# jcatalang/LUDVM

Measured on AMD Instinct MI355X. Metric: biot_savart_pair_interactions_per_s, higher is better.
Workload: dtype f32

## Files before the change

include/ludvm_hip.h:

```cpp
#ifndef LUDVM_HIP_H
#define LUDVM_HIP_H

#include <stddef.h>

#ifdef __cplusplus
extern "C" {
#endif

#define LUDVM_ABI_VERSION 7

enum {
  LUDVM_OK = 0,
  LUDVM_E_ARG = 1,
  LUDVM_E_HIP = 2,
  LUDVM_E_NOMEM = 3,
  LUDVM_E_NODEVICE = 4,
  LUDVM_E_STATE = 5,
  LUDVM_E_COMM = 6
};

enum {
  LUDVM_PREC_F32 = 0,
  LUDVM_PREC_F32X2 = 1,
  LUDVM_PREC_F64 = 2
// ... 1 lines not shown

typedef struct ludvm_ctx ludvm_ctx;


int ludvm_abi_version(void);
int ludvm_create(int device_ordinal, ludvm_ctx** out);
int ludvm_destroy(ludvm_ctx* ctx);
const char* ludvm_last_error(const ludvm_ctx* ctx);
int ludvm_device_info(ludvm_ctx* ctx, int* cu_count, int* clock_khz, long long* hbm_bytes, char* name,
                      int name_len);
int ludvm_set_stream(ludvm_ctx* ctx, void* hip_stream, int external);
int ludvm_synchronize(ludvm_ctx* ctx);
int ludvm_set_tuning(ludvm_ctx* ctx, int targets_per_lane, int source_splits);

int ludvm_set_symmetric(ludvm_ctx* ctx, int mode);
int ludvm_set_sym_tuning(ludvm_ctx* ctx, int vortices_per_lane, int rotation_split);

typedef int (*ludvm_allreduce_fn)(void* user, void* d_buf, size_t count, void* hip_stream);
int ludvm_set_shard(ludvm_ctx* ctx, int rank, int world, size_t min_vortices, ludvm_allreduce_fn allreduce, void* user,
                    void* d_acc, size_t acc_bytes);

#define LUDVM_COMM_ID_BYTES 128
int ludvm_comm_unique_id(void* id_out, size_t id_bytes);
int ludvm_comm_init(ludvm_ctx* ctx, int rank, int world, const void* id, size_t id_bytes, size_t min_vortices);
int ludvm_comm_init_all(ludvm_ctx** ctxs, int n, size_t min_vortices);
int ludvm_comm_destroy(ludvm_ctx* ctx);
int ludvm_comm_info(ludvm_ctx* ctx, int* rank, int* world);
int ludvm_comm_allreduce_i64_dev(ludvm_ctx* ctx, long long* d_buf, size_t count);
int ludvm_comm_allgather_dev(ludvm_ctx* ctx, const void* d_send, void* d_recv, size_t bytes_per_rank);
int ludvm_comm_allgather_host(ludvm_ctx* ctx, const void* send, void* recv, size_t bytes_per_rank);
// ... 161 lines not shown
```

ludvm_amd/_ffi.py:

```python
import ctypes
import importlib.util
import os
import sys
from ctypes import POINTER, c_char_p, c_double, c_float, c_int, c_longlong, c_size_t, c_void_p

_HERE = os.path.dirname(os.path.abspath(__file__))
LIB_PATH = os.path.join(_HERE, "csrc", "libludvm_hip.so")
EXP_LIB_PATH = os.path.join(_HERE, "csrc", "libludvm_hip_exp.so")

OK, E_ARG, E_HIP, E_NOMEM, E_NODEVICE, E_STATE, E_COMM = range(7)
PREC_F32, PREC_F32X2, PREC_F64 = 0, 1, 2
SYM_TILE = 512
SYM_OWNER_ALIGN = 4
ABI_VERSION = 7
COMM_ID_BYTES = 128
ENSEMBLE_MAX_STEPS = 2048
ENSEMBLE_MAX_WAKE = 8192
ENSEMBLE_MAX_SNAPSHOTS = 1024
ENSEMBLE_INIT_HEAD = 8
ENSEMBLE_DESC = 6
ENSEMBLE_MAX_PROBES = 1024
ENSEMBLE_PROBE_BYTES = 1 << 30
ENSEMBLE_MAX_TRACERS = 4096
ENSEMBLE_TRACER_BYTES = 1 << 30
# ... 10 lines not shown
SURVEY_F32_PER_LANE = 4
SYM_SCALE_BYTES = 32

_pd, _pf = POINTER(c_double), POINTER(c_float)

SIGNATURES = {
    "ludvm_abi_version": [],
    "ludvm_create": [c_int, POINTER(c_void_p)],
    "ludvm_destroy": [c_void_p],
    "ludvm_last_error": [c_void_p],
    "ludvm_device_info": [c_void_p, POINTER(c_int), POINTER(c_int), POINTER(c_longlong), c_char_p, c_int],
    "ludvm_set_stream": [c_void_p, c_void_p, c_int],
    "ludvm_synchronize": [c_void_p],
    "ludvm_set_tuning": [c_void_p, c_int, c_int],
    "ludvm_set_symmetric": [c_void_p, c_int],
    "ludvm_set_shard": [c_void_p, c_int, c_int, c_size_t, c_void_p, c_void_p, c_void_p, c_size_t],
    "ludvm_set_sym_tuning": [c_void_p, c_int, c_int],
    "ludvm_comm_unique_id": [c_void_p, c_size_t],
    "ludvm_comm_init": [c_void_p, c_int, c_int, c_void_p, c_size_t, c_size_t],
    "ludvm_comm_init_all": [POINTER(c_void_p), c_int, c_size_t],
    "ludvm_comm_destroy": [c_void_p],
    "ludvm_comm_info": [c_void_p, POINTER(c_int), POINTER(c_int)],
    "ludvm_comm_allreduce_i64_dev": [c_void_p, c_void_p, c_size_t],
    "ludvm_comm_allgather_dev": [c_void_p, c_void_p, c_void_p, c_size_t],
    "ludvm_comm_allgather_host": [c_void_p, c_void_p, c_void_p, c_size_t],
    "ludvm_induce_f64": [c_void_p, _pd, _pd, _pd, c_size_t, _pd, _pd, c_size_t, c_double, c_int, _pd, _pd],
    "ludvm_spatial_order": [c_void_p, _pd, _pd, c_size_t, POINTER(ctypes.c_uint), POINTER(c_int), _pd],
    "ludvm_induce_f32": [c_void_p, _pf, _pf, _pf, c_size_t, _pf, _pf, c_size_t, c_float, _pf, _pf],
    "ludvm_induce_dev_f32": [c_void_p, c_void_p, c_void_p, c_void_p, c_size_t, c_void_p, c_void_p, c_size_t,
                             c_float, c_void_p, c_void_p],
# ... 142 lines not shown
```

ludvm_amd/csrc/context.hip:

```cpp
#include "ctx.hpp"

namespace ludvm_host {

int fail(ludvm_ctx* c, int code, const std::string& msg) {
  if (c) c->err = msg;
  return code;
}

int fail_hip(ludvm_ctx* c, const char* what, hipError_t e) {
  return fail(c, e == hipErrorOutOfMemory ? LUDVM_E_NOMEM : LUDVM_E_HIP,
              std::string(what) + ": " + hipGetErrorString(e));
}

int ensure(ludvm_ctx* c, Buf& b, size_t bytes) {
  if (bytes <= b.cap) return LUDVM_OK;
  HIPCHK(c, hipStreamSynchronize(c->stream));
  if (c->stream_b) HIPCHK(c, hipStreamSynchronize(c->stream_b));
  if (b.p) HIPCHK(c, hipFree(b.p));
  b.p = nullptr;
  b.cap = 0;
  size_t want = std::max(bytes, (size_t)1 << 20);
  HIPCHK(c, hipMalloc(&b.p, want));
  b.cap = want;
  return LUDVM_OK;
// ... 173 lines not shown
  c->shard_min_n = (long long)min_vortices;
  c->reduce_hook = world > 1 ? allreduce : nullptr;
  c->reduce_user = user;
  c->ext_acc = world > 1 ? d_acc : nullptr;
  c->ext_acc_bytes = world > 1 ? acc_bytes : 0;
  return LUDVM_OK;
}

int ludvm_set_symmetric(ludvm_ctx* c, int mode) {
  if (!c) return LUDVM_E_ARG;
  if (mode < 0) return fail(c, LUDVM_E_ARG, "symmetric mode must be >= 0");
  c->sym_mode = mode;
  return LUDVM_OK;
}

}
```

ludvm_amd/csrc/ctx.hpp:

```cpp
#pragma once
#pragma GCC visibility push(default)
#include "../../include/ludvm_hip.h"
#pragma GCC visibility pop
#include "pair_kernels.hpp"
#include "pair_sym_kernels.hpp"
#include "march_types.hpp"
#include "spatial_order.hpp"

#include <hip/hip_ext.h>
#include <rccl/rccl.h>
#include <dlfcn.h>

#include <algorithm>
#include <cmath>
#include <cstdio>
#include <cstdlib>
#include <cstring>
#include <string>
#include <utility>
#include <vector>

using namespace ludvm;

#ifdef LUDVM_EXPERIMENTS
// ... 9 lines not shown

struct TimedLaunch {
  hipEvent_t e0, e1;
};

struct ludvm_ctx {
  int device = 0;
  hipStream_t own_stream = nullptr;
  hipStream_t stream = nullptr;
  hipDeviceProp_t prop;
  std::string err;

  int tune_tpl = 0;
  int tune_split = 0;
  int sym_mode = 1;
  int tune_sym_t = 0, tune_sym_rsplit = 0;
  int xcd_run = 0;
  long long sym_tail_items = kSymTailItems;
  int grid_kernel = 2;
  long long small_tile_max = kSmallTileMaxDefault;
  bool sym_quad = true;
  long long sym_quad_min_tiles = kSymQuadMinTiles;
  bool few_packed = true;
  long long small_tile_max_f64 = kSmallTileMaxF64Default;

  Buf part;
  Buf acc;
  Buf symsc;
  Buf arena;
  Buf orderws;
// ... 106 lines not shown
  long long chunk;
  long long nt_pad;
  dim3 grid;
};

Plan make_plan(const ludvm_ctx* c, long long nt_launch, long long ns, int precision, bool small_ok = true, long long plan_nt = 0,
               bool grid_patch = false);
int timed_begin(ludvm_ctx* c, TimedLaunch& t, bool& active);
int timed_end(ludvm_ctx* c, TimedLaunch& t, bool active);
int drain_timing(ludvm_ctx* c);
int launch_pair(ludvm_ctx* c, PairArgs a, const Plan& p, int precision, void* u, void* w);
int induce_device(ludvm_ctx* c, const PairArgs& a, long long nt, long long ns, int precision, void* u, void* w,
                  long long plan_nt = 0);
long long sym_threshold(const ludvm_ctx* c, bool march = false);
bool use_symmetric(const ludvm_ctx* c, long long n, double vc4, bool march = false);
int sym_tile_t(const ludvm_ctx* c, long long n, bool hilo);

struct SymOperands {
  const float* x; const float* z; const float* g;
  const float* xl = nullptr; const float* zl = nullptr;
  const float* cx = nullptr; const float* cz = nullptr;
  long long* acc_u; long long* acc_w;
  const SymScale* scale; long long* bad;
};

int launch_sym_tiles(ludvm_ctx* c, int T, const SymOperands& o, long long n, long long i_first, long long i_count, double vc4,
                     const long long* n_dev = nullptr, long long n_lo = 0, bool sharded = false);
int acc_buffer(ludvm_ctx* c, long long nt_pad, long long** acc);
bool sharded_at(const ludvm_ctx* c, long long n);
void shard_tiles(const ludvm_ctx* c, long long ntiles, long long* first, long long* count);
// ... 13 lines not shown
  unsigned* order[2];
  double* ext;
  double* sum;
  void* tmp;
  size_t tmp_bytes;
};

int order_workspace(ludvm_ctx* c, size_t nmax, OrderWs* w);
int class_extent_sum(ludvm_ctx* c, const OrderWs& w, const double* dx, const double* dz, const unsigned* order, size_t n, double* out,
                     double* box = nullptr);
int spatial_order_if_needed(ludvm_ctx* c, const OrderWs& w, int slot, const double* dx, const double* dz, size_t n,
                            const unsigned** order_out, double* mean_extent);
int order_gather(ludvm_ctx* c, const double* s0, const double* s1, const double* s2, const unsigned* order, long long n, double* d0,
                 double* d1, double* d2);
int order_scatter(ludvm_ctx* c, const double* s0, const double* s1, const unsigned* order, long long n, double* d0, double* d1);
constexpr double kMaxExtentOverCore = 300.0;
constexpr double kMaxExtentOverCoreCloud = 150.0;
inline bool too_sparse(double mean_extent, bool reordered, double vcore) {
  return vcore > 0.0 && mean_extent > (reordered ? kMaxExtentOverCoreCloud : kMaxExtentOverCore) * vcore;
}

int wake_grow(ludvm_ctx* c, size_t capacity);
int wake_refresh(ludvm_ctx* c, size_t first, size_t count, bool staged = false);
inline unsigned fin_blocks(long long n) { return (unsigned)((n + kFinBlock - 1) / kFinBlock); }
struct MarchSym { const SymScale* scale = nullptr; long long* bad = nullptr; long long n_lo = 0; bool march = false; };
int advect_launch(ludvm_ctx* c, size_t n, const long long* n_dev, double dt, size_t nfoil, double vcore,
                  int precision, double* du, double* dw, TailDuty td = TailDuty{}, MarchSym ms = MarchSym{});

}

// ... 2 lines not shown
```

ludvm_amd/csrc/induce.hip:

```cpp
#include "ctx.hpp"
#include "induce_kernels.hpp"

extern "C" {


int ludvm_induce_f64(ludvm_ctx* c, const double* xs, const double* zs, const double* gs, size_t ns, const double* xt,
                     const double* zt, size_t nt, double vcore, int precision, double* u, double* w) {
  if (!c) return LUDVM_E_ARG;
  if (!valid_precision(precision)) return fail(c, LUDVM_E_ARG, "unknown precision");
  if ((ns && (!xs || !zs || !gs)) || (nt && (!xt || !zt || !u || !w))) return fail(c, LUDVM_E_ARG, "null array");
  if (nt == 0) return LUDVM_OK;
  HIPCHK(c, hipSetDevice(c->device));
  if (ns == 0) {
    std::memset(u, 0, nt * sizeof(double));
    std::memset(w, 0, nt * sizeof(double));
    return LUDVM_OK;
  }
  if (precision == LUDVM_PREC_F32 && std::min(ns, nt) < kOrderMin)
    precision = (double)ns * (double)nt <= kSmallSidePairsF64 ? LUDVM_PREC_F64 : LUDVM_PREC_F32X2;
  const bool f64 = precision == LUDVM_PREC_F64;
  bool hilo = precision == LUDVM_PREC_F32X2;
  const bool self = xt == xs && zt == zs && nt == ns;
  const size_t ntu = self ? 0 : nt;
  const size_t in_doubles = 3 * ns + 2 * ntu, out_doubles = 2 * nt;
// ... 77 lines not shown
    if (hilo)
      hipLaunchKernelGGL(cvt_packed_inputs, dim3(blocks_for((long long)in_doubles)), dim3(kBlock), 0, c->stream, din,
                         (long long)ns, (long long)ntu, fxs, fxsl, fzs, fzsl, fgs, fxt, fxtl, fzt, fztl);
    else
      hipLaunchKernelGGL(cvt_packed_inputs_local, dim3(blocks_for((long long)in_doubles)), dim3(kBlock), 0, c->stream, din,
                         (long long)ns, (long long)ntu, fxs, fzs, fgs, sox, soz, fxt, fzt, tox, toz);
    HIPCHK(c, hipGetLastError());
    if (self && use_symmetric(c, (long long)ns, a.vc4)) {
      long long nt_pad = 0;
      SymOperands o{};
      o.x = fxs; o.z = fzs; o.g = fgs;
      if (hilo) { o.xl = fxsl; o.zl = fzsl; } else { o.cx = sox; o.cz = soz; }
      const long long *acc = nullptr, *bad = nullptr;
      CHK(launch_sym(c, o, (long long)ns, a.vc4, &nt_pad, &acc, &bad));
      hipLaunchKernelGGL(finish_sym, dim3(blocks_for((long long)nt)), dim3(kBlock), 0, c->stream, acc, acc + nt_pad, ctx_scale(c),
                         bad, (long long)nt, fu, fw);
      HIPCHK(c, hipGetLastError());
    } else {
      a.xs = fxs; a.zs = fzs; a.gs = fgs;
      a.xt = self ? fxs : fxt; a.zt = self ? fzs : fzt;
      if (hilo) {
        a.xsl = fxsl; a.zsl = fzsl;
        a.xtl = self ? fxsl : fxtl; a.ztl = self ? fzsl : fztl;
      } else {
        a.scx = sox; a.scz = soz;
        a.tcx = self ? sox : tox; a.tcz = self ? soz : toz;
        a.t_index0 = 0;
      }
      CHK(induce_device(c, a, (long long)nt, (long long)ns, hilo ? LUDVM_PREC_F32X2 : LUDVM_PREC_F32, fu, fw));
    }
    hipLaunchKernelGGL(cvt_packed_outputs, dim3(blocks_for((long long)out_doubles)), dim3(kBlock), 0, c->stream, fu, fw, dout,
// ... 46 lines not shown
  HIPCHK(c, hipMemcpyAsync(u, du, nt * 4, hipMemcpyDeviceToHost, c->stream));
  HIPCHK(c, hipMemcpyAsync(w, dw, nt * 4, hipMemcpyDeviceToHost, c->stream));
  HIPCHK(c, hipStreamSynchronize(c->stream));
  return LUDVM_OK;
}

int ludvm_induce_dev_f32(ludvm_ctx* c, const float* d_xs, const float* d_zs, const float* d_gs, size_t ns,
                         const float* d_xt, const float* d_zt, size_t nt, float vcore, float* d_u, float* d_w) {
  if (!c) return LUDVM_E_ARG;
  if ((ns && (!d_xs || !d_zs || !d_gs)) || (nt && (!d_xt || !d_zt || !d_u || !d_w)))
    return fail(c, LUDVM_E_ARG, "null array");
  HIPCHK(c, hipSetDevice(c->device));
  const double v2 = (double)vcore * (double)vcore;
  if (d_xt == d_xs && d_zt == d_zs && nt == ns && use_symmetric(c, (long long)ns, v2 * v2)) {
    long long nt_pad = 0;
    SymOperands o{};
    o.x = d_xs; o.z = d_zs; o.g = d_gs;
    const long long *acc = nullptr, *bad = nullptr;
    CHK(launch_sym(c, o, (long long)ns, v2 * v2, &nt_pad, &acc, &bad));
    hipLaunchKernelGGL(finish_sym, dim3(blocks_for((long long)nt)), dim3(kBlock), 0, c->stream, acc, acc + nt_pad, ctx_scale(c),
                       bad, (long long)nt, d_u, d_w);
    HIPCHK(c, hipGetLastError());
    return LUDVM_OK;
  }
  PairArgs a{};
  a.xs = d_xs; a.zs = d_zs; a.gs = d_gs; a.ns = (long long)ns;
  a.xt = d_xt; a.zt = d_zt; a.nt = (long long)nt;
  a.vc4 = v2 * v2;
  return induce_device(c, a, (long long)nt, (long long)ns, LUDVM_PREC_F32, d_u, d_w);
}

int ludvm_advect_dev_f32(ludvm_ctx* c, const float* d_xs, const float* d_zs, const float* d_gs, size_t ns,
                         size_t t_first, size_t nt, float vcore, float dt, float* d_x_out, float* d_z_out) {
  if (!c) return LUDVM_E_ARG;
  if (!d_xs || !d_zs || !d_gs || !d_x_out || !d_z_out) return fail(c, LUDVM_E_ARG, "null array");
  if (t_first + nt > ns) return fail(c, LUDVM_E_ARG, "target range outside the source arrays");
  if (nt == 0) return LUDVM_OK;
  HIPCHK(c, hipSetDevice(c->device));
  const double v2 = (double)vcore * (double)vcore;
  if (t_first == 0 && nt == ns && use_symmetric(c, (long long)ns, v2 * v2)) {
    long long nt_pad = 0;
    SymOperands o{};
    o.x = d_xs; o.z = d_zs; o.g = d_gs;
    const long long *acc = nullptr, *bad = nullptr;
    CHK(launch_sym(c, o, (long long)ns, v2 * v2, &nt_pad, &acc, &bad));
    hipLaunchKernelGGL(finish_sym_advect, dim3(blocks_for((long long)nt)), dim3(kBlock), 0, c->stream, acc, acc + nt_pad,
                       ctx_scale(c), bad, d_xs, d_zs, 0LL, (long long)nt, dt, d_x_out, d_z_out);
    HIPCHK(c, hipGetLastError());
    return LUDVM_OK;
  }
  PairArgs a{};
  a.xs = d_xs; a.zs = d_zs; a.gs = d_gs; a.ns = (long long)ns;
  a.xt = d_xs + t_first; a.zt = d_zs + t_first; a.nt = (long long)nt;
  a.vc4 = v2 * v2;
  Plan p = make_plan(c, (long long)nt, (long long)ns, LUDVM_PREC_F32);
  CHK(launch_pair(c, a, p, LUDVM_PREC_F32, nullptr, nullptr));
  hipLaunchKernelGGL(finish_advect_f32, dim3(blocks_for((long long)nt)), dim3(kBlock), 0, c->stream,
                     static_cast<const float*>(c->part.p), (long long)nt, p.nt_pad, p.nsplit, d_xs, d_zs,
                     (long long)t_first, dt, d_x_out, d_z_out);
  HIPCHK(c, hipGetLastError());
  return LUDVM_OK;
}
// ... 23 lines not shown
  o.x = d_x; o.z = d_z; o.g = d_g;
  o.acc_u = d_acc_u; o.acc_w = d_acc_w;
  o.scale = static_cast<const SymScale*>(d_scale);
  o.bad = d_bad;
  return launch_sym_tiles(c, 8, o, (long long)n, (long long)tile_first, (long long)tile_count, v2 * v2);
}

int ludvm_advect_from_sums_dev_f32(ludvm_ctx* c, const long long* d_sum_u, const long long* d_sum_w, const void* d_scale,
                                   const long long* d_bad, const float* d_x, const float* d_z, size_t t_first, size_t nt,
                                   float dt, float* d_x_out, float* d_z_out) {
  if (!c) return LUDVM_E_ARG;
  if (!d_sum_u || !d_sum_w || !d_scale || !d_bad || !d_x || !d_z || !d_x_out || !d_z_out) return fail(c, LUDVM_E_ARG, "null array");
  if (nt == 0) return LUDVM_OK;
  HIPCHK(c, hipSetDevice(c->device));
  hipLaunchKernelGGL(finish_sym_advect, dim3(blocks_for((long long)nt)), dim3(kBlock), 0, c->stream, d_sum_u, d_sum_w,
                     static_cast<const SymScale*>(d_scale), d_bad, d_x, d_z, (long long)t_first, (long long)nt, dt, d_x_out,
                     d_z_out);
  HIPCHK(c, hipGetLastError());
  return LUDVM_OK;
}

}
```

ludvm_amd/csrc/induce_kernels.hpp:

```cpp
#pragma once
#include "pair_kernels.hpp"
#include "pair_sym_kernels.hpp"

namespace ludvm {

__global__ void __launch_bounds__(kBlock)
finish_advect_f32(const float* part, long long nt, long long nt_pad, int nsplit, const float* x, const float* z,
                  long long t_first, float dt, float* x_out, float* z_out) {
  const long long i = (long long)blockIdx.x * kBlock + threadIdx.x;
  if (i >= nt) return;
  float su, sw;
  sum_splits(part, i, nt_pad, nsplit, su, sw);
  x_out[i] = __builtin_fmaf(dt, su, x[t_first + i]);
  z_out[i] = __builtin_fmaf(dt, sw, z[t_first + i]);
}

__global__ void __launch_bounds__(kBlock)
cvt_packed_inputs(const double* in, long long ns, long long nt, float* xs, float* xsl, float* zs, float* zsl, float* gs,
                  float* xt, float* xtl, float* zt, float* ztl) {
  const long long k = (long long)blockIdx.x * kBlock + threadIdx.x;
  if (k >= 3 * ns + 2 * nt) return;
  const double v = in[k];
  float h, l;
  split_hilo(v, h, l);
// ... 22 lines not shown
  if (k < ns) local(0, k, ns, xs, sox);
  else if (k < 2 * ns) local(ns, k - ns, ns, zs, soz);
  else if (k < 3 * ns) gs[k - 2 * ns] = (float)v;
  else if (k < 3 * ns + nt) local(3 * ns, k - 3 * ns, nt, xt, tox);
  else local(3 * ns + nt, k - 3 * ns - nt, nt, zt, toz);
}

__global__ void __launch_bounds__(kBlock)
cvt_packed_outputs(const float* u, const float* w, double* out, long long nt) {
  const long long k = (long long)blockIdx.x * kBlock + threadIdx.x;
  if (k >= 2 * nt) return;
  out[k] = k < nt ? (double)u[k] : (double)w[k - nt];
}

__global__ void __launch_bounds__(kBlock)
finish_sym(const long long* acc_u, const long long* acc_w, const SymScale* sc, const long long* bad, long long n, float* u,
           float* w) {
  const long long i = (long long)blockIdx.x * kBlock + threadIdx.x;
  if (i >= n) return;
  const float s = (float)kInv2PiD;
  u[i] = fx_read(acc_u, i, sc, bad) * s;
  w[i] = -fx_read(acc_w, i, sc, bad) * s;
}

__global__ void __launch_bounds__(kBlock)
finish_sym_advect(const long long* sum_u, const long long* sum_w, const SymScale* sc, const long long* bad, const float* x,
                  const float* z, long long t_first, long long nt, float dt, float* x_out, float* z_out) {
  const long long i = (long long)blockIdx.x * kBlock + threadIdx.x;
  if (i >= nt) return;
  const float s = (float)kInv2PiD;
  x_out[i] = __builtin_fmaf(dt, fx_read(sum_u, i, sc, bad) * s, x[t_first + i]);
  z_out[i] = __builtin_fmaf(dt, -fx_read(sum_w, i, sc, bad) * s, z[t_first + i]);
}

}
```

ludvm_amd/csrc/launch.hip:

```cpp
#include "ctx.hpp"
#include "sym_prepare_kernels.hpp"

namespace ludvm_host {

PlanKnobs plan_knobs(const ludvm_ctx* c) {
  PlanKnobs k;
  k.small_tile_max = c->small_tile_max;
  k.small_tile_max_f64 = c->small_tile_max_f64;
  k.tune_tpl = c->tune_tpl;
  k.tune_split = c->tune_split;
  k.grid_kernel = c->grid_kernel;
  k.few_packed = c->few_packed;
  return k;
}
static_assert(kPlanF32 == LUDVM_PREC_F32 && kPlanF32X2 == LUDVM_PREC_F32X2 && kPlanF64 == LUDVM_PREC_F64, "plan_rule.hpp takes the ABI's precision codes");

Plan make_plan(const ludvm_ctx* c, long long nt_launch, long long ns, int precision, bool small_ok, long long plan_nt, bool grid_patch) {
  const DirectPlan d = direct_plan(plan_knobs(c), nt_launch, ns, precision, small_ok, plan_nt, grid_patch);
  Plan p{};
  p.tpl = d.tpl;
  p.tile = d.tile;
  p.nsplit = d.nsplit;
  p.chunk = d.chunk;
  p.nt_pad = d.nt_pad;
// ... 110 lines not shown
                         static_cast<double*>(w));
    else
      hipLaunchKernelGGL(finish_sum<float>, dim3(blocks_for(nt)), dim3(kBlock), 0, c->stream,
                         static_cast<const float*>(c->part.p), nt, p.nt_pad, p.nsplit, static_cast<float*>(u),
                         static_cast<float*>(w));
    HIPCHK(c, hipGetLastError());
  }
  return LUDVM_OK;
}

static_assert(64 * 8 == LUDVM_SYM_TILE, "the multi-GPU entry points always use the 512-vortex tile");

SymKnobs sym_knobs(const ludvm_ctx* c) {
  SymKnobs k;
  k.sym_mode = c->sym_mode;
  k.tile_t = c->tune_sym_t;
  k.tune_split = c->tune_split;
  k.tune_rsplit = c->tune_sym_rsplit;
  k.quad = c->sym_quad;
  k.quad_min_tiles = c->sym_quad_min_tiles;
  k.tail_items = c->sym_tail_items;
  return k;
}
long long sym_threshold(const ludvm_ctx* c, bool march) { return sym_min_n(sym_knobs(c), march); }
bool use_symmetric(const ludvm_ctx* c, long long n, double vc4, bool march) {
  return sym_use(sym_knobs(c), n, (float)vc4 > 0.0f, march);
}
int sym_tile_t(const ludvm_ctx* c, long long n, bool hilo) { return sym_tile(sym_knobs(c), n, hilo); }

int launch_sym_tiles(ludvm_ctx* c, int T, const SymOperands& o, long long n, long long i_first, long long i_count, double vc4,
                     const long long* n_dev, long long n_lo, bool sharded) {
  if (n >= (1LL << 31)) return fail(c, LUDVM_E_ARG, "the symmetric kernel indexes vortices with 32 bits: n < 2^31");
  SymArgs a{};
  a.x = o.x; a.z = o.z; a.g = o.g; a.n = n;
  a.n_dev = n_dev;
  a.xl = o.xl; a.zl = o.zl;
  a.cx = o.cx; a.cz = o.cz;
  const SymKnobs k = sym_knobs(c);
  const SymVariant v = sym_variant(k, n, T, o.xl && o.zl);
  const SymGeom& gm = v.g;
  a.tune_split = k.tune_split;
  a.tune_rsplit = v.tune_rsplit;
// ... 167 lines not shown
```

ludvm_amd/csrc/order.hip:

```cpp
#include "ctx.hpp"
#include "order_kernels.hpp"

namespace ludvm_host {


namespace {

inline size_t up256(size_t b) { return (b + 255) & ~(size_t)255; }

}

int order_workspace(ludvm_ctx* c, size_t nmax, OrderWs* w) {
  const size_t nblk = (nmax + kOriginBlock - 1) / kOriginBlock;
  const size_t tb = spatial_order_temp_bytes(nmax);
  CHK(ensure(c, c->orderws, 2 * up256(nmax * 4) + up256(nblk * 5 * 8) + 256 + tb));
  char* p = static_cast<char*>(c->orderws.p);
  w->order[0] = reinterpret_cast<unsigned*>(p); p += up256(nmax * 4);
  w->order[1] = reinterpret_cast<unsigned*>(p); p += up256(nmax * 4);
  w->ext = reinterpret_cast<double*>(p); p += up256(nblk * 5 * 8);
  w->sum = reinterpret_cast<double*>(p); p += 256;
  w->tmp = p;
  w->tmp_bytes = tb;
  return LUDVM_OK;
}
// ... 38 lines not shown
}

int order_gather(ludvm_ctx* c, const double* s0, const double* s1, const double* s2, const unsigned* order, long long n, double* d0,
                 double* d1, double* d2) {
  hipLaunchKernelGGL(gather_f64, dim3(blocks_for(n)), dim3(kBlock), 0, c->stream, s0, s1, s2, order, n, d0, d1, d2);
  HIPCHK(c, hipGetLastError());
  return LUDVM_OK;
}

int order_scatter(ludvm_ctx* c, const double* s0, const double* s1, const unsigned* order, long long n, double* d0, double* d1) {
  hipLaunchKernelGGL(scatter_f64, dim3(blocks_for(n)), dim3(kBlock), 0, c->stream, s0, s1, order, n, d0, d1);
  HIPCHK(c, hipGetLastError());
  return LUDVM_OK;
}

}

extern "C" {

int ludvm_spatial_order(ludvm_ctx* c, const double* x, const double* z, size_t n, unsigned* order, int* reordered,
                        double* mean_class_extent) {
  if (!c) return LUDVM_E_ARG;
  if (n && (!x || !z || !order)) return fail(c, LUDVM_E_ARG, "null array");
  if (n >= ((size_t)1 << 32)) return fail(c, LUDVM_E_ARG, "too many points");
  if (reordered) *reordered = 0;
  if (mean_class_extent) *mean_class_extent = 0.0;
  for (size_t i = 0; i < n; ++i) order[i] = (unsigned)i;
  if (n < kOrderMin) return LUDVM_OK;
  HIPCHK(c, hipSetDevice(c->device));
  CHK(ensure(c, c->arena, 2 * Arena::need(n, 8)));
// ... 18 lines not shown
```

ludvm_amd/csrc/order_kernels.hpp:

```cpp
#pragma once
#include "pair_kernels.hpp"

namespace ludvm {

__global__ void __launch_bounds__(kOriginBlock)
class_extents(const double* x, const double* z, const unsigned* order, long long n, double* ext) {
  const long long i = (long long)blockIdx.x * kOriginBlock + threadIdx.x;
  double lo_x = 1e300, hi_x = -1e300, lo_z = 1e300, hi_z = -1e300;
  if (i < n) {
    const long long p = order ? (long long)order[i] : i;
    const double vx = x[p], vz = z[p];
    if (fabs(vx) < 1e300 && fabs(vz) < 1e300) { lo_x = hi_x = vx; lo_z = hi_z = vz; }
  }
  for (int s = 2; s < 64; s <<= 1) {
    lo_x = fmin(lo_x, __shfl_xor(lo_x, s)); hi_x = fmax(hi_x, __shfl_xor(hi_x, s));
    lo_z = fmin(lo_z, __shfl_xor(lo_z, s)); hi_z = fmax(hi_z, __shfl_xor(hi_z, s));
  }
  __shared__ double red[kOriginBlock / 64][2][4];
  const int lane = threadIdx.x & 63, wv = threadIdx.x >> 6;
  if (lane < 2) { red[wv][lane][0] = lo_x; red[wv][lane][1] = hi_x; red[wv][lane][2] = lo_z; red[wv][lane][3] = hi_z; }
  __syncthreads();
  if (threadIdx.x == 0) {
    double e = 0.0, bx0 = 1e300, bx1 = -1e300, bz0 = 1e300, bz1 = -1e300;
    for (int p = 0; p < 2; ++p) {
// ... 18 lines not shown
  }
  __shared__ double red[256][5];
  red[threadIdx.x][0] = s; red[threadIdx.x][1] = x0; red[threadIdx.x][2] = x1; red[threadIdx.x][3] = z0; red[threadIdx.x][4] = z1;
  __syncthreads();
  for (int h = 128; h > 0; h >>= 1) {
    if ((int)threadIdx.x < h) {
      double* a = red[threadIdx.x];
      const double* b = red[threadIdx.x + h];
      a[0] += b[0]; a[1] = fmin(a[1], b[1]); a[2] = fmax(a[2], b[2]); a[3] = fmin(a[3], b[3]); a[4] = fmax(a[4], b[4]);
    }
    __syncthreads();
  }
  if (threadIdx.x < 5) out[threadIdx.x] = red[0][threadIdx.x];
}

__global__ void __launch_bounds__(kBlock)
gather_f64(const double* s0, const double* s1, const double* s2, const unsigned* order, long long n, double* d0, double* d1,
           double* d2) {
  const long long k = (long long)blockIdx.x * kBlock + threadIdx.x;
  if (k >= n) return;
  const long long p = order ? (long long)order[k] : k;
  if (s0) d0[k] = s0[p];
  if (s1) d1[k] = s1[p];
  if (s2) d2[k] = s2[p];
}

__global__ void __launch_bounds__(kBlock)
scatter_f64(const double* s0, const double* s1, const unsigned* order, long long n, double* d0, double* d1) {
  const long long k = (long long)blockIdx.x * kBlock + threadIdx.x;
  if (k >= n) return;
// ... 7 lines not shown
```

ludvm_amd/csrc/spatial_order.hip:

```cpp
#include "spatial_order.hpp"

#include <cstring>

#include <rocprim/device/device_radix_sort.hpp>

namespace ludvm {

namespace {

__device__ __forceinline__ unsigned spread16(unsigned v) {
  v = (v | (v << 8)) & 0x00ff00ffu;
  v = (v | (v << 4)) & 0x0f0f0f0fu;
  v = (v | (v << 2)) & 0x33333333u;
  v = (v | (v << 1)) & 0x55555555u;
  return v;
}

__global__ void __launch_bounds__(256) morton_keys(const double* x, const double* z, unsigned n, OrderBox b, unsigned* keys,
                                                   unsigned* vals) {
  const unsigned i = blockIdx.x * 256u + threadIdx.x;
  if (i >= n) return;
  const double cx = fmin(fmax((x[i] - b.x0) * b.sx, 0.0), 65535.0);
  const double cz = fmin(fmax((z[i] - b.z0) * b.sz, 0.0), 65535.0);
  keys[i] = spread16((unsigned)cx) | (spread16((unsigned)cz) << 1);
  vals[i] = i;
}

inline size_t align256(size_t b) { return (b + 255) & ~(size_t)255; }

size_t rocprim_bytes(size_t n) {
  size_t bytes = 0;
  (void)rocprim::radix_sort_pairs(nullptr, bytes, static_cast<unsigned*>(nullptr), static_cast<unsigned*>(nullptr),
                                  static_cast<unsigned*>(nullptr), static_cast<unsigned*>(nullptr), n, 0, 32, hipStream_t(nullptr));
  return bytes;
}

}

size_t spatial_order_temp_bytes(size_t n) { return 3 * align256(n * sizeof(unsigned)) + align256(rocprim_bytes(n)) + 256; }

hipError_t spatial_order_sort(const double* d_x, const double* d_z, size_t n, OrderBox box, void* d_tmp, size_t tmp_bytes,
                              unsigned* d_order, hipStream_t stream) {
  if (n == 0) return hipSuccess;
  if (n >= (size_t)1 << 32 || tmp_bytes < spatial_order_temp_bytes(n)) return hipErrorInvalidValue;
  char* p = static_cast<char*>(d_tmp);
  unsigned* keys = reinterpret_cast<unsigned*>(p); p += align256(n * sizeof(unsigned));
  unsigned* keys_out = reinterpret_cast<unsigned*>(p); p += align256(n * sizeof(unsigned));
  unsigned* vals = reinterpret_cast<unsigned*>(p); p += align256(n * sizeof(unsigned));
  size_t rp = rocprim_bytes(n);
  hipLaunchKernelGGL(morton_keys, dim3((unsigned)((n + 255) / 256)), dim3(256), 0, stream, d_x, d_z, (unsigned)n, box, keys, vals);
  hipError_t e = hipGetLastError();
  if (e != hipSuccess) return e;
  return rocprim::radix_sort_pairs(p, rp, keys, keys_out, vals, d_order, n, 0, 32, stream);
}

}
```

ludvm_amd/csrc/spatial_order.hpp:

```cpp
#pragma once
#include <hip/hip_runtime.h>

#include <cstddef>

namespace ludvm {

struct OrderBox {
  double x0, z0, sx, sz;
};

size_t spatial_order_temp_bytes(size_t n);

hipError_t spatial_order_sort(const double* d_x, const double* d_z, size_t n, OrderBox box, void* d_tmp, size_t tmp_bytes,
                              unsigned* d_order, hipStream_t stream);

}
```

ludvm_amd/csrc/sym_rule.hpp:

```cpp
#pragma once
#include <cstddef>
#include <cstdio>
#ifndef __HIPCC__
#define __host__
#define __device__
#endif

namespace ludvm {

constexpr long long kSymTargetWaves = 8 * 65536;
constexpr long long kSymMaxSplit = 64;
constexpr long long kSymMaxSplitTuned = 1024;
constexpr long long kXcds = 8;
constexpr long long kSymMaxRsplit = 4;
constexpr long long kSymMinItems = 10500;
constexpr long long kSymTailItems = 1536;
struct SymGeom { long long ntiles, dmax, dtot; int ysplit, rsplit, ytail, rbulk; };
struct XcdShare { unsigned lo, n; };
__host__ __device__ inline XcdShare xcd_share(unsigned units, unsigned e) {
  const unsigned lo = (unsigned)((unsigned long long)units * e / (unsigned)kXcds);
  return XcdShare{lo, (unsigned)((unsigned long long)units * (e + 1) / (unsigned)kXcds) - lo};
}
__host__ __device__ inline unsigned xcd_run(unsigned ys, int k) {
  return k > 0 ? (unsigned)k : (ys > 0 ? (ys + (unsigned)kXcds - 1) / (unsigned)kXcds : 1);
// ... 155 lines not shown
}
__host__ __device__ inline long long quad_blocks(long long i_count, int ysplit, int k = 0) {
  const unsigned quads = (unsigned)((i_count + kQuad - 1) / kQuad);
  long long most = 0;
  for (unsigned x = 0; x < (unsigned)kXcds; ++x) {
    const long long wg = (long long)xcd_items(quads, (unsigned)ysplit, x, 0, (unsigned)ysplit, k);
    most = wg > most ? wg : most;
  }
  return kXcds * most;
}

constexpr long long kSymMinN = 16384;
constexpr long long kSymT8MinN = 36864;
constexpr long long kSymMinNMarch = 11264;
constexpr long long kSymQuadMinTiles = 640;

struct SymKnobs {
  int sym_mode = 1;
  int tile_t = 0;
  int tune_split = 0;
  int tune_rsplit = 0;
  bool quad = true;
  long long quad_min_tiles = kSymQuadMinTiles;
  long long tail_items = kSymTailItems;
  long long t8_min_n = kSymT8MinN;
};

inline long long sym_min_n(const SymKnobs& k, bool march) {
  return k.sym_mode == 1 ? (march ? kSymMinNMarch : kSymMinN) : (long long)k.sym_mode;
}
inline bool sym_use(const SymKnobs& k, long long n, bool core, bool march) {
  return k.sym_mode != 0 && core && n >= sym_min_n(k, march);
}
inline int sym_tile(const SymKnobs& k, long long n, bool hilo) {
  if (hilo) return 4;
  if (k.tile_t == 4 || k.tile_t == 8) return k.tile_t;
  return n >= k.t8_min_n ? 8 : 4;
}

struct SymVariant {
  int T;
  bool hilo;
  int tune_rsplit;
  SymGeom g;
  bool quad;
  QuadGeom q;
};
// ... 32 lines not shown
```

ludvm_amd/engine.py:

```python
import ctypes
from ctypes import POINTER, byref, c_double, c_float, c_int, c_longlong, c_size_t, c_void_p

import numpy as np

from . import _ffi
from ._ffi import PREC_F32, PREC_F32X2, PREC_F64, LudvmHipError

PRECISIONS = {"f32": PREC_F32, "f32x2": PREC_F32X2, "f64": PREC_F64}


def _f64(a):
    return np.ascontiguousarray(a, dtype=np.float64).reshape(-1)


def _f32(a):
    return np.ascontiguousarray(a, dtype=np.float32).reshape(-1)


def _pd(a):
    return a.ctypes.data_as(POINTER(c_double)) if a is not None else None


def _pf(a):
    return a.ctypes.data_as(POINTER(c_float)) if a is not None else None
# ... 56 lines not shown
            self._check(self._lib.ludvm_set_stream(self._ctx, None, 0))
        else:
            self._check(self._lib.ludvm_set_stream(self._ctx, c_void_p(int(hip_stream)), 1))

    def synchronize(self):
        self._check(self._lib.ludvm_synchronize(self._ctx))

    def set_tuning(self, targets_per_lane=0, source_splits=0):
        self._check(self._lib.ludvm_set_tuning(self._ctx, int(targets_per_lane), int(source_splits)))

    def set_sym_tuning(self, vortices_per_lane=0, rotation_split=0):
        self._check(self._lib.ludvm_set_sym_tuning(self._ctx, int(vortices_per_lane), int(rotation_split)))

    def set_symmetric(self, mode=1):
        self._check(self._lib.ludvm_set_symmetric(self._ctx, int(mode)))

    def set_shard(self, rank, world, allreduce=None, d_acc=0, acc_bytes=0, min_vortices=0):
        if world > 1:
            def hook(_user, _buf, count, stream):
                try:
                    allreduce(int(count), int(stream or 0))
                    return 0
                except Exception as e:
                    self._hook_error = e
                    return 1
            self._hook_c = _ffi.ALLREDUCE_FN(hook)
            self._check(self._lib.ludvm_set_shard(self._ctx, int(rank), int(world), int(min_vortices),
                                                  ctypes.cast(self._hook_c, c_void_p), None, c_void_p(int(d_acc)),
                                                  int(acc_bytes)))
        else:
# ... 508 lines not shown
```

Baseline: 8888 billion.

## Morton-reorder device f32 self-interaction inputs before symmetric pair kernel

For large device-resident self-induction (n at or above 524288 by default), the code computes a bounding box on device, builds Morton keys, radix-sorts them, gathers x/z/gamma into sorted order, runs the symmetric kernel on the sorted data, and scatters the results back in the finish kernels. The aim is better spatial locality, which could help tile culling or fixed-point scaling and cache reuse in the symmetric pair kernel. In exchange it adds a sort, a gather and indirect writes on every call, plus extra workspace memory. A knob lets callers turn it off or force it on.

```diff
diff --git a/include/ludvm_hip.h b/include/ludvm_hip.h
--- a/include/ludvm_hip.h
+++ b/include/ludvm_hip.h
@@ -39,6 +39,7 @@
 int ludvm_set_tuning(ludvm_ctx* ctx, int targets_per_lane, int source_splits);
 
 int ludvm_set_symmetric(ludvm_ctx* ctx, int mode);
+int ludvm_set_self_order(ludvm_ctx* ctx, int mode);
 int ludvm_set_sym_tuning(ludvm_ctx* ctx, int vortices_per_lane, int rotation_split);
 
 typedef int (*ludvm_allreduce_fn)(void* user, void* d_buf, size_t count, void* hip_stream);
diff --git a/ludvm_amd/_ffi.py b/ludvm_amd/_ffi.py
--- a/ludvm_amd/_ffi.py
+++ b/ludvm_amd/_ffi.py
@@ -48,6 +48,7 @@
     "ludvm_synchronize": [c_void_p],
     "ludvm_set_tuning": [c_void_p, c_int, c_int],
     "ludvm_set_symmetric": [c_void_p, c_int],
+    "ludvm_set_self_order": [c_void_p, c_int],
     "ludvm_set_shard": [c_void_p, c_int, c_int, c_size_t, c_void_p, c_void_p, c_void_p, c_size_t],
     "ludvm_set_sym_tuning": [c_void_p, c_int, c_int],
     "ludvm_comm_unique_id": [c_void_p, c_size_t],
diff --git a/ludvm_amd/csrc/context.hip b/ludvm_amd/csrc/context.hip
--- a/ludvm_amd/csrc/context.hip
+++ b/ludvm_amd/csrc/context.hip
@@ -211,4 +211,11 @@
   return LUDVM_OK;
 }
 
-}
+int ludvm_set_self_order(ludvm_ctx* c, int mode) {
+  if (!c) return LUDVM_E_ARG;
+  if (mode < 0 || mode > 2) return fail(c, LUDVM_E_ARG, "self-order mode must be 0 (never), 1 (by size) or 2 (always)");
+  c->self_order = mode;
+  return LUDVM_OK;
+}
+
+}
diff --git a/ludvm_amd/csrc/ctx.hpp b/ludvm_amd/csrc/ctx.hpp
--- a/ludvm_amd/csrc/ctx.hpp
+++ b/ludvm_amd/csrc/ctx.hpp
@@ -47,6 +47,7 @@
   int tune_tpl = 0;
   int tune_split = 0;
   int sym_mode = 1;
+  int self_order = 1;
   int tune_sym_t = 0, tune_sym_rsplit = 0;
   int xcd_run = 0;
   long long sym_tail_items = kSymTailItems;
@@ -183,6 +184,7 @@
                   long long plan_nt = 0);
 long long sym_threshold(const ludvm_ctx* c, bool march = false);
 bool use_symmetric(const ludvm_ctx* c, long long n, double vc4, bool march = false);
+bool use_self_order(const ludvm_ctx* c, long long n);
 int sym_tile_t(const ludvm_ctx* c, long long n, bool hilo);
 
 struct SymOperands {
@@ -226,6 +228,11 @@
 int order_gather(ludvm_ctx* c, const double* s0, const double* s1, const double* s2, const unsigned* order, long long n, double* d0,
                  double* d1, double* d2);
 int order_scatter(ludvm_ctx* c, const double* s0, const double* s1, const unsigned* order, long long n, double* d0, double* d1);
+struct SelfOrdered {
+  const unsigned* order;
+  const float *x, *z, *g;
+};
+int self_order_f32(ludvm_ctx* c, const float* d_x, const float* d_z, const float* d_g, size_t n, SelfOrdered* out);
 constexpr double kMaxExtentOverCore = 300.0;
 constexpr double kMaxExtentOverCoreCloud = 150.0;
 inline bool too_sparse(double mean_extent, bool reordered, double vcore) {
diff --git a/ludvm_amd/csrc/induce.hip b/ludvm_amd/csrc/induce.hip
--- a/ludvm_amd/csrc/induce.hip
+++ b/ludvm_amd/csrc/induce.hip
@@ -1,5 +1,23 @@
 #include "ctx.hpp"
 #include "induce_kernels.hpp"
+
+namespace {
+
+int sym_self_dev(ludvm_ctx* c, const float* d_x, const float* d_z, const float* d_g, long long n, double vc4, long long* nt_pad,
+                 const long long** acc, const long long** bad, const unsigned** order) {
+  SymOperands o{};
+  o.x = d_x; o.z = d_z; o.g = d_g;
+  *order = nullptr;
+  if (use_self_order(c, n)) {
+    SelfOrdered so{};
+    CHK(self_order_f32(c, d_x, d_z, d_g, (size_t)n, &so));
+    o.x = so.x; o.z = so.z; o.g = so.g;
+    *order = so.order;
+  }
+  return launch_sym(c, o, n, vc4, nt_pad, acc, bad);
+}
+
+}
 
 extern "C" {
 
@@ -115,7 +133,7 @@
       const long long *acc = nullptr, *bad = nullptr;
       CHK(launch_sym(c, o, (long long)ns, a.vc4, &nt_pad, &acc, &bad));
       hipLaunchKernelGGL(finish_sym, dim3(blocks_for((long long)nt)), dim3(kBlock), 0, c->stream, acc, acc + nt_pad, ctx_scale(c),
-                         bad, (long long)nt, fu, fw);
+                         bad, (const unsigned*)nullptr, (long long)nt, fu, fw);
       HIPCHK(c, hipGetLastError());
     } else {
       a.xs = fxs; a.zs = fzs; a.gs = fgs;
@@ -192,12 +210,11 @@
   const double v2 = (double)vcore * (double)vcore;
   if (d_xt == d_xs && d_zt == d_zs && nt == ns && use_symmetric(c, (long long)ns, v2 * v2)) {
     long long nt_pad = 0;
-    SymOperands o{};
-    o.x = d_xs; o.z = d_zs; o.g = d_gs;
     const long long *acc = nullptr, *bad = nullptr;
-    CHK(launch_sym(c, o, (long long)ns, v2 * v2, &nt_pad, &acc, &bad));
+    const unsigned* order = nullptr;
+    CHK(sym_self_dev(c, d_xs, d_zs, d_gs, (long long)ns, v2 * v2, &nt_pad, &acc, &bad, &order));
     hipLaunchKernelGGL(finish_sym, dim3(blocks_for((long long)nt)), dim3(kBlock), 0, c->stream, acc, acc + nt_pad, ctx_scale(c),
-                       bad, (long long)nt, d_u, d_w);
+                       bad, order, (long long)nt, d_u, d_w);
     HIPCHK(c, hipGetLastError());
     return LUDVM_OK;
   }
@@ -218,12 +235,11 @@
   const double v2 = (double)vcore * (double)vcore;
   if (t_first == 0 && nt == ns && use_symmetric(c, (long long)ns, v2 * v2)) {
     long long nt_pad = 0;
-    SymOperands o{};
-    o.x = d_xs; o.z = d_zs; o.g = d_gs;
     const long long *acc = nullptr, *bad = nullptr;
-    CHK(launch_sym(c, o, (long long)ns, v2 * v2, &nt_pad, &acc, &bad));
+    const unsigned* order = nullptr;
+    CHK(sym_self_dev(c, d_xs, d_zs, d_gs, (long long)ns, v2 * v2, &nt_pad, &acc, &bad, &order));
     hipLaunchKernelGGL(finish_sym_advect, dim3(blocks_for((long long)nt)), dim3(kBlock), 0, c->stream, acc, acc + nt_pad,
-                       ctx_scale(c), bad, d_xs, d_zs, 0LL, (long long)nt, dt, d_x_out, d_z_out);
+                       ctx_scale(c), bad, order, d_xs, d_zs, 0LL, (long long)nt, dt, d_x_out, d_z_out);
     HIPCHK(c, hipGetLastError());
     return LUDVM_OK;
   }
@@ -277,8 +293,8 @@
   if (nt == 0) return LUDVM_OK;
   HIPCHK(c, hipSetDevice(c->device));
   hipLaunchKernelGGL(finish_sym_advect, dim3(blocks_for((long long)nt)), dim3(kBlock), 0, c->stream, d_sum_u, d_sum_w,
-                     static_cast<const SymScale*>(d_scale), d_bad, d_x, d_z, (long long)t_first, (long long)nt, dt, d_x_out,
-                     d_z_out);
+                     static_cast<const SymScale*>(d_scale), d_bad, (const unsigned*)nullptr, d_x, d_z, (long long)t_first,
+                     (long long)nt, dt, d_x_out, d_z_out);
   HIPCHK(c, hipGetLastError());
   return LUDVM_OK;
 }
diff --git a/ludvm_amd/csrc/induce_kernels.hpp b/ludvm_amd/csrc/induce_kernels.hpp
--- a/ludvm_amd/csrc/induce_kernels.hpp
+++ b/ludvm_amd/csrc/induce_kernels.hpp
@@ -60,23 +60,25 @@
 }
 
 __global__ void __launch_bounds__(kBlock)
-finish_sym(const long long* acc_u, const long long* acc_w, const SymScale* sc, const long long* bad, long long n, float* u,
-           float* w) {
+finish_sym(const long long* acc_u, const long long* acc_w, const SymScale* sc, const long long* bad, const unsigned* order,
+           long long n, float* u, float* w) {
   const long long i = (long long)blockIdx.x * kBlock + threadIdx.x;
   if (i >= n) return;
+  const long long p = order ? (long long)order[i] : i;
   const float s = (float)kInv2PiD;
-  u[i] = fx_read(acc_u, i, sc, bad) * s;
-  w[i] = -fx_read(acc_w, i, sc, bad) * s;
+  u[p] = fx_read(acc_u, i, sc, bad) * s;
+  w[p] = -fx_read(acc_w, i, sc, bad) * s;
 }
 
 __global__ void __launch_bounds__(kBlock)
-finish_sym_advect(const long long* sum_u, const long long* sum_w, const SymScale* sc, const long long* bad, const float* x,
-                  const float* z, long long t_first, long long nt, float dt, float* x_out, float* z_out) {
+finish_sym_advect(const long long* sum_u, const long long* sum_w, const SymScale* sc, const long long* bad, const unsigned* order,
+                  const float* x, const float* z, long long t_first, long long nt, float dt, float* x_out, float* z_out) {
   const long long i = (long long)blockIdx.x * kBlock + threadIdx.x;
   if (i >= nt) return;
+  const long long p = order ? (long long)order[i] : i;
   const float s = (float)kInv2PiD;
-  x_out[i] = __builtin_fmaf(dt, fx_read(sum_u, i, sc, bad) * s, x[t_first + i]);
-  z_out[i] = __builtin_fmaf(dt, -fx_read(sum_w, i, sc, bad) * s, z[t_first + i]);
+  x_out[p] = __builtin_fmaf(dt, fx_read(sum_u, i, sc, bad) * s, x[t_first + p]);
+  z_out[p] = __builtin_fmaf(dt, -fx_read(sum_w, i, sc, bad) * s, z[t_first + p]);
 }
 
 }
diff --git a/ludvm_amd/csrc/launch.hip b/ludvm_amd/csrc/launch.hip
--- a/ludvm_amd/csrc/launch.hip
+++ b/ludvm_amd/csrc/launch.hip
@@ -148,6 +148,7 @@
 SymKnobs sym_knobs(const ludvm_ctx* c) {
   SymKnobs k;
   k.sym_mode = c->sym_mode;
+  k.self_order = c->self_order;
   k.tile_t = c->tune_sym_t;
   k.tune_split = c->tune_split;
   k.tune_rsplit = c->tune_sym_rsplit;
@@ -160,6 +161,7 @@
 bool use_symmetric(const ludvm_ctx* c, long long n, double vc4, bool march) {
   return sym_use(sym_knobs(c), n, (float)vc4 > 0.0f, march);
 }
+bool use_self_order(const ludvm_ctx* c, long long n) { return sym_self_order(sym_knobs(c), n); }
 int sym_tile_t(const ludvm_ctx* c, long long n, bool hilo) { return sym_tile(sym_knobs(c), n, hilo); }
 
 int launch_sym_tiles(ludvm_ctx* c, int T, const SymOperands& o, long long n, long long i_first, long long i_count, double vc4,
diff --git a/ludvm_amd/csrc/order.hip b/ludvm_amd/csrc/order.hip
--- a/ludvm_amd/csrc/order.hip
+++ b/ludvm_amd/csrc/order.hip
@@ -76,6 +76,29 @@
   return LUDVM_OK;
 }
 
+int self_order_f32(ludvm_ctx* c, const float* d_x, const float* d_z, const float* d_g, size_t n, SelfOrdered* out) {
+  if (n >= ((size_t)1 << 32)) return fail(c, LUDVM_E_ARG, "too many points");
+  const long long nblk = (long long)((n + kBoxChunk - 1) / kBoxChunk);
+  const size_t tb = spatial_order_temp_bytes(n), nb = up256(n * 4);
+  CHK(ensure(c, c->orderws, 4 * nb + up256((size_t)nblk * 4 * sizeof(float)) + 256 + tb));
+  char* p = static_cast<char*>(c->orderws.p);
+  unsigned* order = reinterpret_cast<unsigned*>(p); p += nb;
+  float* xo = reinterpret_cast<float*>(p); p += nb;
+  float* zo = reinterpret_cast<float*>(p); p += nb;
+  float* go = reinterpret_cast<float*>(p); p += nb;
+  float* part = reinterpret_cast<float*>(p); p += up256((size_t)nblk * 4 * sizeof(float));
+  OrderBox* box = reinterpret_cast<OrderBox*>(p); p += 256;
+  hipLaunchKernelGGL(box_partial_f32, dim3((unsigned)nblk), dim3(256), 0, c->stream, d_x, d_z, (long long)n, part);
+  hipLaunchKernelGGL(box_final_f32, dim3(1), dim3(256), 0, c->stream, part, nblk, box);
+  HIPCHK(c, hipGetLastError());
+  HIPCHK(c, spatial_order_sort_f32(d_x, d_z, n, box, p, tb, order, c->stream));
+  hipLaunchKernelGGL(gather_f32, dim3(blocks_for((long long)n)), dim3(kBlock), 0, c->stream, d_x, d_z, d_g, order, (long long)n, xo,
+                     zo, go);
+  HIPCHK(c, hipGetLastError());
+  *out = SelfOrdered{order, xo, zo, go};
+  return LUDVM_OK;
+}
+
 }
 
 extern "C" {
diff --git a/ludvm_amd/csrc/order_kernels.hpp b/ludvm_amd/csrc/order_kernels.hpp
--- a/ludvm_amd/csrc/order_kernels.hpp
+++ b/ludvm_amd/csrc/order_kernels.hpp
@@ -1,5 +1,6 @@
 #pragma once
 #include "pair_kernels.hpp"
+#include "spatial_order.hpp"
 
 namespace ludvm {
 
@@ -56,6 +57,62 @@
   if (threadIdx.x < 5) out[threadIdx.x] = red[0][threadIdx.x];
 }
 
+constexpr int kBoxChunk = 4096;
+__device__ __forceinline__ void box_merge(float& x0, float& x1, float& z0, float& z1, float a, float b, float c, float d) {
+  x0 = __builtin_fminf(x0, a); x1 = __builtin_fmaxf(x1, b); z0 = __builtin_fminf(z0, c); z1 = __builtin_fmaxf(z1, d);
+}
+__device__ __forceinline__ void box_reduce_block(float& x0, float& x1, float& z0, float& z1) {
+  for (int s = 1; s < 64; s <<= 1)
+    box_merge(x0, x1, z0, z1, __shfl_xor(x0, s), __shfl_xor(x1, s), __shfl_xor(z0, s), __shfl_xor(z1, s));
+  __shared__ float red[4][4];
+  const int lane = threadIdx.x & 63, wv = threadIdx.x >> 6;
+  if (lane == 0) { red[wv][0] = x0; red[wv][1] = x1; red[wv][2] = z0; red[wv][3] = z1; }
+  __syncthreads();
+  if (threadIdx.x == 0)
+    for (int w = 1; w < 4; ++w) box_merge(x0, x1, z0, z1, red[w][0], red[w][1], red[w][2], red[w][3]);
+}
+__global__ void __launch_bounds__(256) box_partial_f32(const float* x, const float* z, long long n, float* part) {
+  const float inf = __builtin_inff();
+  float x0 = inf, x1 = -inf, z0 = inf, z1 = -inf;
+  const long long base = (long long)blockIdx.x * kBoxChunk;
+  for (int j = 0; j < kBoxChunk / 256; ++j) {
+    const long long i = base + j * 256 + threadIdx.x;
+    if (i < n) {
+      const float vx = x[i], vz = z[i];
+      if (__builtin_fabsf(vx) < inf && __builtin_fabsf(vz) < inf) box_merge(x0, x1, z0, z1, vx, vx, vz, vz);
+    }
+  }
+  box_reduce_block(x0, x1, z0, z1);
+  if (threadIdx.x == 0) {
+    float* o = part + 4 * (long long)blockIdx.x;
+    o[0] = x0; o[1] = x1; o[2] = z0; o[3] = z1;
+  }
+}
+__global__ void __launch_bounds__(256) box_final_f32(const float* part, long long nblk, OrderBox* box) {
+  const float inf = __builtin_inff();
+  float x0 = inf, x1 = -inf, z0 = inf, z1 = -inf;
+  for (long long i = threadIdx.x; i < nblk; i += 256) box_merge(x0, x1, z0, z1, part[4 * i], part[4 * i + 1], part[4 * i + 2], part[4 * i + 3]);
+  box_reduce_block(x0, x1, z0, z1);
+  if (threadIdx.x == 0) {
+    const bool any = x1 >= x0;
+    const double ex = any ? (double)x1 - (double)x0 : 0.0, ez = any ? (double)z1 - (double)z0 : 0.0;
+    box->x0 = any ? (double)x0 : 0.0;
+    box->z0 = any ? (double)z0 : 0.0;
+    box->sx = ex > 0.0 ? 65536.0 / ex : 0.0;
+    box->sz = ez > 0.0 ? 65536.0 / ez : 0.0;
+  }
+}
+
+__global__ void __launch_bounds__(kBlock)
+gather_f32(const float* x, const float* z, const float* g, const unsigned* order, long long n, float* xo, float* zo, float* go) {
+  const long long k = (long long)blockIdx.x * kBlock + threadIdx.x;
+  if (k >= n) return;
+  const long long p = (long long)order[k];
+  xo[k] = x[p];
+  zo[k] = z[p];
+  go[k] = g[p];
+}
+
 __global__ void __launch_bounds__(kBlock)
 gather_f64(const double* s0, const double* s1, const double* s2, const unsigned* order, long long n, double* d0, double* d1,
            double* d2) {
diff --git a/ludvm_amd/csrc/spatial_order.hip b/ludvm_amd/csrc/spatial_order.hip
--- a/ludvm_amd/csrc/spatial_order.hip
+++ b/ludvm_amd/csrc/spatial_order.hip
@@ -26,6 +26,22 @@
   vals[i] = i;
 }
 
+__global__ void __launch_bounds__(256) morton_keys_f32(const float* x, const float* z, unsigned n, const OrderBox* box,
+                                                       unsigned* keys, unsigned* vals) {
+  const unsigned i = blockIdx.x * 256u + threadIdx.x;
+  if (i >= n) return;
+  const OrderBox b = *box;
+  const float vx = x[i], vz = z[i];
+  unsigned key = 0xffffffffu;
+  if (__builtin_fabsf(vx) < __builtin_inff() && __builtin_fabsf(vz) < __builtin_inff()) {
+    const double cx = fmin(fmax(((double)vx - b.x0) * b.sx, 0.0), 65535.0);
+    const double cz = fmin(fmax(((double)vz - b.z0) * b.sz, 0.0), 65535.0);
+    key = spread16((unsigned)cx) | (spread16((unsigned)cz) << 1);
+  }
+  keys[i] = key;
+  vals[i] = i;
+}
+
 inline size_t align256(size_t b) { return (b + 255) & ~(size_t)255; }
 
 size_t rocprim_bytes(size_t n) {
@@ -39,8 +55,10 @@
 
 size_t spatial_order_temp_bytes(size_t n) { return 3 * align256(n * sizeof(unsigned)) + align256(rocprim_bytes(n)) + 256; }
 
-hipError_t spatial_order_sort(const double* d_x, const double* d_z, size_t n, OrderBox box, void* d_tmp, size_t tmp_bytes,
-                              unsigned* d_order, hipStream_t stream) {
+namespace {
+
+template <typename LaunchKeys>
+hipError_t sort_by_keys(size_t n, void* d_tmp, size_t tmp_bytes, unsigned* d_order, hipStream_t stream, LaunchKeys launch_keys) {
   if (n == 0) return hipSuccess;
   if (n >= (size_t)1 << 32 || tmp_bytes < spatial_order_temp_bytes(n)) return hipErrorInvalidValue;
   char* p = static_cast<char*>(d_tmp);
@@ -48,10 +66,27 @@
   unsigned* keys_out = reinterpret_cast<unsigned*>(p); p += align256(n * sizeof(unsigned));
   unsigned* vals = reinterpret_cast<unsigned*>(p); p += align256(n * sizeof(unsigned));
   size_t rp = rocprim_bytes(n);
-  hipLaunchKernelGGL(morton_keys, dim3((unsigned)((n + 255) / 256)), dim3(256), 0, stream, d_x, d_z, (unsigned)n, box, keys, vals);
+  launch_keys(keys, vals);
   hipError_t e = hipGetLastError();
   if (e != hipSuccess) return e;
   return rocprim::radix_sort_pairs(p, rp, keys, keys_out, vals, d_order, n, 0, 32, stream);
 }
 
 }
+
+hipError_t spatial_order_sort(const double* d_x, const double* d_z, size_t n, OrderBox box, void* d_tmp, size_t tmp_bytes,
+                              unsigned* d_order, hipStream_t stream) {
+  return sort_by_keys(n, d_tmp, tmp_bytes, d_order, stream, [&](unsigned* keys, unsigned* vals) {
+    hipLaunchKernelGGL(morton_keys, dim3((unsigned)((n + 255) / 256)), dim3(256), 0, stream, d_x, d_z, (unsigned)n, box, keys, vals);
+  });
+}
+
+hipError_t spatial_order_sort_f32(const float* d_x, const float* d_z, size_t n, const OrderBox* d_box, void* d_tmp,
+                                  size_t tmp_bytes, unsigned* d_order, hipStream_t stream) {
+  return sort_by_keys(n, d_tmp, tmp_bytes, d_order, stream, [&](unsigned* keys, unsigned* vals) {
+    hipLaunchKernelGGL(morton_keys_f32, dim3((unsigned)((n + 255) / 256)), dim3(256), 0, stream, d_x, d_z, (unsigned)n, d_box, keys,
+                       vals);
+  });
+}
+
+}
diff --git a/ludvm_amd/csrc/spatial_order.hpp b/ludvm_amd/csrc/spatial_order.hpp
--- a/ludvm_amd/csrc/spatial_order.hpp
+++ b/ludvm_amd/csrc/spatial_order.hpp
@@ -14,4 +14,7 @@
 hipError_t spatial_order_sort(const double* d_x, const double* d_z, size_t n, OrderBox box, void* d_tmp, size_t tmp_bytes,
                               unsigned* d_order, hipStream_t stream);
 
+hipError_t spatial_order_sort_f32(const float* d_x, const float* d_z, size_t n, const OrderBox* d_box, void* d_tmp,
+                                  size_t tmp_bytes, unsigned* d_order, hipStream_t stream);
+
 }
diff --git a/ludvm_amd/csrc/sym_rule.hpp b/ludvm_amd/csrc/sym_rule.hpp
--- a/ludvm_amd/csrc/sym_rule.hpp
+++ b/ludvm_amd/csrc/sym_rule.hpp
@@ -193,9 +193,11 @@
 constexpr long long kSymT8MinN = 36864;
 constexpr long long kSymMinNMarch = 11264;
 constexpr long long kSymQuadMinTiles = 640;
+constexpr long long kSelfOrderMin = 524288;
 
 struct SymKnobs {
   int sym_mode = 1;
+  int self_order = 1;
   int tile_t = 0;
   int tune_split = 0;
   int tune_rsplit = 0;
@@ -210,6 +212,9 @@
 }
 inline bool sym_use(const SymKnobs& k, long long n, bool core, bool march) {
   return k.sym_mode != 0 && core && n >= sym_min_n(k, march);
+}
+inline bool sym_self_order(const SymKnobs& k, long long n) {
+  return k.self_order == 2 || (k.self_order == 1 && n >= kSelfOrderMin);
 }
 inline int sym_tile(const SymKnobs& k, long long n, bool hilo) {
   if (hilo) return 4;
diff --git a/ludvm_amd/engine.py b/ludvm_amd/engine.py
--- a/ludvm_amd/engine.py
+++ b/ludvm_amd/engine.py
@@ -94,6 +94,9 @@
 
     def set_symmetric(self, mode=1):
         self._check(self._lib.ludvm_set_symmetric(self._ctx, int(mode)))
+
+    def set_self_order(self, mode=1):
+        self._check(self._lib.ludvm_set_self_order(self._ctx, int(mode)))
 
     def set_shard(self, rank, world, allreduce=None, d_acc=0, acc_bytes=0, min_vortices=0):
         if world > 1:
```

New measurement: 9141 billion (median of 6 runs). +2.8%, better.
